# PhilippKath/concentus

Hardware: NVIDIA B200
Metric: CELT decode audio-sec per sec (x realtime), 48k stereo (higher is better)
Workload: dtype int32

## Files before the change

concentus_b200/csrc/celt_arith.cuh:

```cuda
#pragma once
#include "celt_simt.cuh"

namespace cb {

typedef int16_t s16_t;

CB_DEV int s16(int x) { return (int)(int16_t)x; }
CB_DEV int imin(int a, int b) { return a < b ? a : b; }
CB_DEV int imax(int a, int b) { return a > b ? a : b; }
CB_DEV int iabs(int a) { return a < 0 ? -a : a; }
CB_DEV int wadd(int a, int b) { return (int)((unsigned)a + (unsigned)b); }
CB_DEV int wsub(int a, int b) { return (int)((unsigned)a - (unsigned)b); }
CB_DEV int wmul(int a, int b) { return (int)((unsigned)a * (unsigned)b); }
CB_DEV int wneg(int a) { return (int)(0u - (unsigned)a); }

CB_DEV int ec_ilog(unsigned x) { return 32 - CB_CLZ(x); }

CB_DEV int shl32(int a, int s) { return (int)((unsigned)a << s); }
CB_DEV int shr32(int a, int s) { return a >> s; }
CB_DEV int pshr32(int a, int s) { return wadd(a, (1 << s) >> 1) >> s; }
CB_DEV int vshr32(int a, int s) { return s > 0 ? (a >> s) : shl32(a, -s); }
CB_DEV int shl16(int a, int s) { return s16((int)((unsigned)(uint16_t)a << s)); }
CB_DEV int round16(int a, int s) { return s16(pshr32(a, s)); }
CB_DEV int sat16(int x) { return x > 32767 ? 32767 : (x < -32768 ? -32768 : x); }

CB_DEV int mul16_16(int a, int b) { return s16(a) * s16(b); }
CB_DEV int mac16_16(int c, int a, int b) { return wadd(c, s16(a) * s16(b)); }
CB_DEV int mul16_16_q15(int a, int b) { return mul16_16(a, b) >> 15; }
CB_DEV int mul16_16_q14(int a, int b) { return mul16_16(a, b) >> 14; }
CB_DEV int mul16_16_q13(int a, int b) { return mul16_16(a, b) >> 13; }
CB_DEV int mul16_16_q11(int a, int b) { return mul16_16(a, b) >> 11; }
CB_DEV int mul16_16_p15(int a, int b) { return wadd(16384, mul16_16(a, b)) >> 15; }
CB_DEV int mul16_16_p14(int a, int b) { return wadd(8192, mul16_16(a, b)) >> 14; }
CB_DEV int mul16_16_p13(int a, int b) { return wadd(4096, mul16_16(a, b)) >> 13; }

CB_DEV int mul16_32_q15(int a, int b) { return (int)(((int64_t)s16(a) * (int64_t)b) >> 15); }
CB_DEV int mul16_32_q16(int a, int b) { return (int)(((int64_t)s16(a) * (int64_t)b) >> 16); }
CB_DEV int mul16_32_p16(int a, int b) { return (int)(((int64_t)s16(a) * (int64_t)b + 32768) >> 16); }
CB_DEV int mul32_32_q31(int a, int b) {
    int ah = a >> 16, bh = b >> 16;
    int al = a & 0xffff, bl = b & 0xffff;
    int t0 = shl32(s16(ah) * s16(bh), 1);
    int t1 = (s16(ah) * bl) >> 15;
    int t2 = (s16(bh) * al) >> 15;
    return wadd(wadd(t0, t1), t2);
}
CB_DEV int mac16_32_q15(int c, int a, int b) {
    return wadd(c, wadd(s16(a) * s16(b >> 15), (s16(a) * (b & 0x7fff)) >> 15));
}
CB_DEV int frac_mul16(int a, int b) { return (16384 + s16(a) * s16(b)) >> 15; }
CB_DEV int sig2word16(int x) { return sat16(pshr32(x, 12)); }

CB_DEV int celt_ilog2(int x) { return ec_ilog((unsigned)x) - 1; }
CB_DEV int celt_zlog2(int x) { return x <= 0 ? 0 : celt_ilog2(x); }

CB_MATH unsigned isqrt32(unsigned v) {
    unsigned g = 0;
    int bshift = (ec_ilog(v) - 1) >> 1;
    unsigned b = 1u << bshift;
    do {
        unsigned t = ((g << 1) + b) << bshift;
        if (t <= v) { g += b; v -= t; }
        b >>= 1;
        bshift--;
    } while (bshift >= 0);
    return g;
}

CB_MATH int celt_rcp(int x) {
    int i = celt_ilog2(x);
    int n = s16(vshr32(x, i - 15) - 32768);
    int r = s16(30840 + mul16_16_q15(-15420, n));
    r = s16(r - mul16_16_q15(r, s16(mul16_16_q15(r, n) + s16(r - 32768))));
    r = s16(r - s16(1 + mul16_16_q15(r, s16(mul16_16_q15(r, n) + s16(r - 32768)))));
    return vshr32(r, i - 16);
}
CB_DEV int celt_div(int a, int b) { return mul32_32_q31(a, celt_rcp(b)); }

CB_MATH int frac_div32(int a, int b) {
    int shift = celt_ilog2(b) - 29;
    a = vshr32(a, shift);
    b = vshr32(b, shift);
    int rcp = round16(celt_rcp(round16(b, 16)), 3);
    int result = mul16_32_q15(rcp, a);
    int rem = wsub(pshr32(a, 2), mul32_32_q31(result, b));
    result = wadd(result, shl32(mul16_32_q15(rcp, rem), 2));
    if (result >= 536870912) return 2147483647;
    if (result <= -536870912) return -2147483647;
    return shl32(result, 2);
}

CB_MATH int celt_rsqrt_norm(int x) {
    int n = s16(x - 32768);
    int r = s16(23557 + mul16_16_q15(n, s16(-13490 + mul16_16_q15(n, 6713))));
    int r2 = s16(mul16_16_q15(r, r));
    int y = shl16(s16(s16(mul16_16_q15(r2, n) + r2)) - 16384, 1);
    return s16(r + mul16_16_q15(r, s16(mul16_16_q15(y, s16(s16(mul16_16_q15(y, 12288)) - 16384)))));
}

CB_MATH int celt_sqrt(int x) {
    if (x == 0) return 0;
    if (x >= 1073741824) return 32767;
    int k = (celt_ilog2(x) >> 1) - 7;
    x = vshr32(x, 2 * k);
    int n = s16(x - 32768);
    int rt = s16(23175 + mul16_16_q15(n, s16(11561 + mul16_16_q15(n, s16(-3011 +
              mul16_16_q15(n, s16(1699 + mul16_16_q15(n, -664))))))));
    return vshr32(rt, 7 - k);
}

CB_MATH int celt_cos_pi_2(int x) {
    int x2 = s16(mul16_16_p15(x, x));
    int inner = wadd(-7651, mul16_16_p15(x2, wadd(8277, mul16_16_p15(-626, x2))));
    int v = wadd((32767 - x2), mul16_16_p15(x2, inner));
    return s16(1 + imin(32766, v));
}
CB_MATH int celt_cos_norm(int x) {
    x = x & 0x0001ffff;
    if (x > (1 << 16)) x = (1 << 17) - x;
    if (x & 0x00007fff) {
        if (x < (1 << 15)) return celt_cos_pi_2(s16(x));
        return s16(-celt_cos_pi_2(s16(65536 - x)));
    }
    if (x & 0x0000ffff) return 0;
    if (x & 0x0001ffff) return -32767;
    return 32767;
}

CB_MATH int celt_log2(int x) {
    if (x == 0) return -32767;
    int i = celt_ilog2(x);
    int n = s16(vshr32(x, i - 15) - 32768 - 16384);
    int frac = s16(-6793 + mul16_16_q15(n, s16(15746 + mul16_16_q15(n, s16(-5217 +
                mul16_16_q15(n, s16(2545 + mul16_16_q15(n, -1401))))))));
    return s16(shl16(i - 13, 10) + (frac >> 4));
}

CB_DEV int celt_exp2_frac(int x) {
    int frac = shl16(x, 4);
    return s16(16383 + mul16_16_q15(frac, s16(22804 + mul16_16_q15(frac, s16(14819 + mul16_16_q15(10204, frac))))));
}
CB_MATH int celt_exp2(int x) {
    int integer = s16(x) >> 10;
    if (integer > 14) return 0x7f000000;
    if (integer < -15) return 0;
    int frac = celt_exp2_frac(s16(s16(x) - shl16(integer, 10)));
    return vshr32(frac, -integer - 2);
}

CB_DEV int celt_atan01(int x) {
    return s16(mul16_16_p15(x, wadd(32767, mul16_16_p15(x, wadd(-21, mul16_16_p15(x, wadd(-11943, mul16_16_p15(4936, x))))))));
}
CB_MATH int celt_atan2p(int y, int x) {
    if (y < x) {
        int arg = celt_div(shl32(y, 15), x);
        if (arg >= 32767) arg = 32767;
        return celt_atan01(s16(arg)) >> 1;
    } else {
        int arg = celt_div(shl32(x, 15), y);
        if (arg >= 32767) arg = 32767;
        return 25736 - (celt_atan01(s16(arg)) >> 1);
    }
}

CB_MATH int bitexact_cos(int x) {
    x = s16(x);
    int tmp = (4096 + x * x) >> 13;
    int x2 = s16(tmp);
    x2 = s16((32767 - x2) + frac_mul16(x2, (-7651 + frac_mul16(x2, (8277 + frac_mul16(-626, x2))))));
    return s16(1 + x2);
}
CB_MATH int bitexact_log2tan(int isin, int icos) {
    int lc = ec_ilog((unsigned)icos);
    int ls = ec_ilog((unsigned)isin);
    icos <<= 15 - lc;
    isin <<= 15 - ls;
    return (ls - lc) * (1 << 11) + frac_mul16(isin, frac_mul16(isin, -2597) + 7932)
           - frac_mul16(icos, frac_mul16(icos, -2597) + 7932);
}

CB_DEV unsigned lcg_rand(unsigned seed) { return 1664525u * seed + 1013904223u; }
CB_TABLE uint32_t kLcgMul[23] = {1u, 1664525u, 389569705u, 2940799637u, 158984081u, 2862450781u, 3211393721u, 1851289957u, 3934847009u, 2184914861u, 246739401u, 1948736821u, 2941245873u, 4195587069u, 4088025561u, 980655621u, 2001863745u, 657792333u, 65284841u, 1282409429u, 3808694225u, 2968195997u, 2417331449u};
CB_TABLE uint32_t kLcgAdd[23] = {0u, 1013904223u, 1196435762u, 3519870697u, 2868466484u, 1649599747u, 2670642822u, 1476291629u, 2748932008u, 2180890343u, 2498801434u, 3421909937u, 3167820124u, 2636375307u, 3801544430u, 28987765u, 2210837584u, 3039689583u, 1338634754u, 1649346937u, 2768872580u, 2254235155u, 2326606934u};
CB_DEV unsigned lcg_jump(unsigned seed, int k) { return kLcgMul[k] * seed + kLcgAdd[k]; }

CB_DEV unsigned udiv(unsigned n, unsigned d) { return n / d; }
CB_DEV int sudiv(int n, int d) { return n / d; }

}
```

concentus_b200/csrc/celt_decoder.cuh:

```cuda
#pragma once
#include "celt_bands.cuh"
#include "celt_energy.cuh"
#include "celt_ir.h"
#include "celt_mdct.cuh"
#include "opus_state.h"


namespace cb {


struct ParseScratch {
    int16_t norm[2 * 8 * 78];
    alignas(16) int16_t tmp[176];
    alignas(16) int16_t xw[2 * 176];
    alignas(16) int16_t lbs[176];
};

CB_DEV void celt_parse_frame(const uint8_t *data, int len, int LM, int C, int end, unsigned *seed, CbFrameIR &ir, int16_t *X,
                             ParseScratch &ps, bool dry) {
    const int start = 0;
    const int M = 1 << LM;
    const int N = M * kShortMdct;
    int tf_res[kNbEBands], cap[kNbEBands], offsets[kNbEBands], fine_quant[kNbEBands], pulses[kNbEBands], fine_priority[kNbEBands];
    AllocScratch alloc;
    EcDec dec;
    dec.init(data, (unsigned)len);

    int total_bits = len * 8;
    int tell = dec.tell();
    int silence;
    if (tell >= total_bits) silence = 1;
    else if (tell == 1) silence = dec.bit_logp(15);
    else silence = 0;
    if (silence) {
        tell = len * 8;
        dec.nbits_total += tell - dec.tell();
    }
    int postfilter_gain = 0, postfilter_pitch = 0, postfilter_tapset = 0;
    if (start == 0 && tell + 16 <= total_bits) {
        if (dec.bit_logp(1)) {
            int octave = (int)dec.uint_(6);
            postfilter_pitch = (16 << octave) + (int)dec.bits(4 + octave) - 1;
            int qg = (int)dec.bits(3);
            if (dec.tell() + 2 <= total_bits) postfilter_tapset = dec.icdf(kTapsetIcdf, 2);
            postfilter_gain = 3072 * (qg + 1);
        }
        tell = dec.tell();
    }
    int isTransient = 0;
    if (LM > 0 && tell + 3 <= total_bits) {
        isTransient = dec.bit_logp(3);
        tell = dec.tell();
    }
    const int shortBlocks = isTransient ? M : 0;
    const int intra_ener = tell + 3 <= total_bits ? dec.bit_logp(3) : 0;
    CB_NOUNROLL for (int i = 0; i < 2 * kNbEBands; i++) { ir.qi[i] = 0; ir.eoff[i] = 0; }
    decode_coarse_symbols(start, end, intra_ener, dec, C, LM, ir.qi);
    tf_decode(start, end, isTransient, tf_res, LM, dec);
    tell = dec.tell();
    int spread_decision = kSpreadNormal;
    if (tell + 4 <= total_bits) spread_decision = dec.icdf(kSpreadIcdf, 5);
    init_caps(cap, LM, C);
    int dynalloc_logp = 6;
    total_bits <<= kBitRes;
    tell = (int)dec.tell_frac();
    CB_NOUNROLL for (int i = start; i < end; i++) {
        int width = C * band_width(i) << LM;
        int quanta = imin(width << kBitRes, imax(6 << kBitRes, width));
        int loop_logp = dynalloc_logp;
        int boost = 0;
        while (tell + (loop_logp << kBitRes) < total_bits && boost < cap[i]) {
            int flag = dec.bit_logp(loop_logp);
            tell = (int)dec.tell_frac();
            if (!flag) break;
            boost += quanta;
            total_bits -= quanta;
            loop_logp = 1;
        }
        offsets[i] = boost;
        if (boost > 0) dynalloc_logp = imax(2, dynalloc_logp - 1);
    }
    int alloc_trim = tell + (6 << kBitRes) <= total_bits ? dec.icdf(kTrimIcdf, 7) : 5;
    int bits = ((len * 8) << kBitRes) - (int)dec.tell_frac() - 1;
    int anti_collapse_rsv = isTransient && LM >= 2 && bits >= ((LM + 2) << kBitRes) ? (1 << kBitRes) : 0;
    bits -= anti_collapse_rsv;
    int intensity = 0, dual_stereo = 0, balance = 0;
    AllocDecIo io{dec};
    int codedBands = compute_allocation(io, alloc, start, end, offsets, cap, alloc_trim, &intensity, &dual_stereo, bits, &balance,
                                        pulses, fine_quant, fine_priority, C, LM);
    decode_fine_energy(start, end, fine_quant, dec, C, ir.eoff);

    unsigned sd = *seed;
    quant_all_bands_dec(start, end, X, C == 2 ? X + N : nullptr, ir.collapse, pulses, shortBlocks, spread_decision, dual_stereo,
                        intensity, tf_res, len * (8 << kBitRes) - anti_collapse_rsv, balance, dec, LM, codedBands, &sd, ps.norm,
                        ps.tmp, ps.xw, ps.lbs, dry);
    int anti_collapse_on = 0;
    if (anti_collapse_rsv > 0) anti_collapse_on = (int)dec.bits(1);
    decode_energy_finalise(start, end, fine_quant, fine_priority, len * 8 - dec.tell(), dec, C, ir.eoff);

    ir.rng_final = dec.rng;
    ir.seed_bands = sd;
    ir.len = (int16_t)len;
    ir.pf_pitch = (int16_t)postfilter_pitch;
    ir.pf_gain = (int16_t)postfilter_gain;
    ir.pf_tapset = (uint8_t)postfilter_tapset;
    ir.LM = (uint8_t)LM; ir.C = (uint8_t)C; ir.end = (uint8_t)end;
    ir.flags = (uint8_t)((silence ? CB_IR_SILENCE : 0) | (isTransient ? CB_IR_TRANSIENT : 0) | (intra_ener ? CB_IR_INTRA : 0) |
                         (anti_collapse_on ? CB_IR_ANTICOLLAPSE : 0) | (dec.error ? CB_IR_EC_ERROR : 0) |
                         (dec.tell() > 8 * len ? CB_IR_OVERRUN : 0));
    CB_NOUNROLL for (int i = 0; i < kNbEBands; i++) ir.pulses[i] = (int16_t)(i < end ? pulses[i] : 0);
    *seed = dec.rng;
}


struct SynthScratch {
    int fft[kMaxFrame];
    int16_t den_gain[2][kNbEBands];
    int8_t den_shift[2][kNbEBands];
};

template <class TM>
CB_DEV void comb_filter_inplace(TM tm, int *x, int T0, int T1, int N, int g0, int g1, int tapset0, int tapset1, int overlap) {
    if (g0 == 0 && g1 == 0) return;
    const int g00 = s16(mul16_16_p15(g0, kCombGains[tapset0][0]));
    const int g01 = s16(mul16_16_p15(g0, kCombGains[tapset0][1]));
    const int g02 = s16(mul16_16_p15(g0, kCombGains[tapset0][2]));
    const int g10 = s16(mul16_16_p15(g1, kCombGains[tapset1][0]));
    const int g11 = s16(mul16_16_p15(g1, kCombGains[tapset1][1]));
    const int g12 = s16(mul16_16_p15(g1, kCombGains[tapset1][2]));
    if (g0 == g1 && T0 == T1 && tapset0 == tapset1) overlap = 0;
    const int Tmin = imin(g0 != 0 ? T0 : kCombMaxPeriod, g1 != 0 ? T1 : kCombMaxPeriod);
    const int G = imin(TM::W, Tmin - 2);
    CB_NOUNROLL for (int base = 0; base < overlap; base += G) {
        int i = base + tm.lane();
        if (tm.lane() < G && i < overlap) {
            int f = s16(mul16_16_q15(kWindow120[i], kWindow120[i]));
            int nf = 32767 - f;
            int v = x[i];
            if (g0 != 0) {
                v = wadd(v, mul16_32_q15(mul16_16_q15(nf, g00), x[i - T0]));
                v = wadd(v, mul16_32_q15(mul16_16_q15(nf, g01), wadd(x[i - T0 + 1], x[i - T0 - 1])));
                v = wadd(v, mul16_32_q15(mul16_16_q15(nf, g02), wadd(x[i - T0 + 2], x[i - T0 - 2])));
            }
            if (g1 != 0) {
                v = wadd(v, mul16_32_q15(mul16_16_q15(f, g10), x[i - T1]));
                v = wadd(v, mul16_32_q15(mul16_16_q15(f, g11), wadd(x[i - T1 + 1], x[i - T1 - 1])));
                v = wadd(v, mul16_32_q15(mul16_16_q15(f, g12), wadd(x[i - T1 + 2], x[i - T1 - 2])));
            }
            x[i] = v;
        }
        tm.sync();
    }
    if (g1 == 0) return;
    CB_NOUNROLL for (int base = overlap; base < N; base += G) {
        int i = base + tm.lane();
        if (tm.lane() < G && i < N) {
            int v = x[i];
            v = wadd(v, mul16_32_q15(g10, x[i - T1]));
            v = wadd(v, mul16_32_q15(g11, wadd(x[i - T1 + 1], x[i - T1 - 1])));
            v = wadd(v, mul16_32_q15(g12, wadd(x[i - T1 + 2], x[i - T1 - 2])));
            x[i] = v;
        }
        tm.sync();
    }
}

CB_DEV int deemphasis_channel(const int *x, int n, int16_t *y, int CC, int downsample, int m, int gain) {
    if (downsample > 1) {
        int k = 0, next = 0;
        CB_NOUNROLL for (int j = 0; j < n; j++) {
            int t = wadd(x[j], m);
            m = mul16_32_q15(kPreemphCoef0, t);
            if (j == next) {
                int v = sig2word16(t);
                if (gain >= 0) { int g = mul16_32_p16(v, gain); v = g > 32767 ? 32767 : (g < -32767 ? -32767 : g); }
                y[k * CC] = (int16_t)v;
                k++;
                next += downsample;
            }
        }
    } else {
        int j = 0;
        if ((((uintptr_t)x) & 15) == 0) {
            CB_NOUNROLL for (; j + 8 <= n; j += 8) {
                int xs[8];
                const int4 a = *reinterpret_cast<const int4 *>(x + j);
                const int4 b = *reinterpret_cast<const int4 *>(x + j + 4);
                xs[0] = a.x; xs[1] = a.y; xs[2] = a.z; xs[3] = a.w; xs[4] = b.x; xs[5] = b.y; xs[6] = b.z; xs[7] = b.w;
#pragma unroll
                CB_NOUNROLL for (int u = 0; u < 8; u++) {
                    int t = wadd(xs[u], m);
                    m = mul16_32_q15(kPreemphCoef0, t);
                    int v = sig2word16(t);
                    if (gain >= 0) { int g = mul16_32_p16(v, gain); v = g > 32767 ? 32767 : (g < -32767 ? -32767 : g); }
                    y[(j + u) * CC] = (int16_t)v;
                }
            }
        }
        CB_NOUNROLL for (; j < n; j++) {
            int t = wadd(x[j], m);
            m = mul16_32_q15(kPreemphCoef0, t);
            int v = sig2word16(t);
            if (gain >= 0) { int g = mul16_32_p16(v, gain); v = g > 32767 ? 32767 : (g < -32767 ? -32767 : g); }
            y[j * CC] = (int16_t)v;
        }
    }
    return m;
}

template <class TM>
CB_DEV void history_shift(TM tm, int *mem, int N, int count = -1) {
    if (count < 0) count = kDecBuf - N + kOverlap / 2;
    if (((count | N) & 3) == 0) {
        int4 *m4 = reinterpret_cast<int4 *>(mem);
        const int nv = count >> 2, sh = N >> 2;
        CB_NOUNROLL for (int base = 0; base < nv; base += 2 * TM::W) {
            const int i0 = base + tm.lane(), i1 = i0 + TM::W;
            int4 a = {0, 0, 0, 0}, b = {0, 0, 0, 0};
            if (i0 < nv) a = m4[i0 + sh];
            if (i1 < nv) b = m4[i1 + sh];
            tm.sync();
            if (i0 < nv) m4[i0] = a;
            if (i1 < nv) m4[i1] = b;
        }
        tm.sync();
        return;
    }
    CB_NOUNROLL for (int base = 0; base < count; base += TM::W) {
        int i = base + tm.lane();
        int v = 0;
        if (i < count) v = mem[i + N];
        tm.sync();
        if (i < count) mem[i] = v;
    }
    tm.sync();
}

template <class TM>
CB_DEV void celt_synthesis_team(TM tm, SynthScratch &S, const int16_t *X, int *const *out_syn, const int16_t *oldBandE, int start, int effEnd,
                                int C, int CC, int isTransient, int LM, int downsample, int silence) {
    const int M = 1 << LM;
    const int N = M * kShortMdct;
    {
        int bstart = start, bend = effEnd;
        int bound = M * kEBands[bend];
        if (downsample != 1) bound = imin(bound, N / downsample);
        if (silence) { bound = 0; bstart = bend = 0; }
        const int lo = M * kEBands[bstart];
        CB_TEAM_FOR(w, C * kNbEBands, tm) {
            int c = w / kNbEBands, i = w - c * kNbEBands;
            int lg = s16(oldBandE[c * kNbEBands + i] + shl16(kEMeans[i], 6));
            int shift = 16 - (lg >> 10);
            int g;
            if (shift > 31) { shift = 0; g = 0; }
            else g = celt_exp2_frac(lg & 1023);
            if (shift < -2) { g = 32767; shift = -2; }
            S.den_gain[c][i] = (int16_t)g;
            S.den_shift[c][i] = (int8_t)shift;
        }
        tm.sync();
        const int B = isTransient ? M : 1;
        const int shift = isTransient ? kMaxLM : kMaxLM - LM;
        const int hi = imin(bound, M * kEBands[bend]);
        auto freq = [&](int mode, int j) -> int {
            if (j < lo || j >= hi) return 0;
            const int b = kBinToBand[j >> LM];
            int v0 = 0, v1 = 0;
            if (mode != 1) {
                int v = mul16_16(X[j], S.den_gain[0][b]);
                int sh = S.den_shift[0][b];
                v0 = sh < 0 ? shl32(v, -sh) : (v >> sh);
            }
            if (mode != 0) {
                int v = mul16_16(X[N + j], S.den_gain[1][b]);
                int sh = S.den_shift[1][b];
                v1 = sh < 0 ? shl32(v, -sh) : (v >> sh);
            }
            return mode == 0 ? v0 : mode == 1 ? v1 : (wadd(v0, v1) >> 1);
        };
        const int npass = (CC == 2 && C == 2) ? 2 : 1;
        CB_NOUNROLL for (int p = 0; p < npass; p++) {
            const int mode = (CC == 1 && C == 2) ? 2 : p;
            imdct_compute(tm, [&](int j) { return freq(mode, j); }, B, shift, S.fft);
            imdct_assemble(tm, out_syn[p], B, shift, S.fft);
            if (CC == 2 && C == 1) imdct_assemble(tm, out_syn[1], B, shift, S.fft);
        }
    }
}

template <class TM>
CB_DEV int celt_synth_frame(TM tm, CbDecState *st, SynthScratch &S, const CbFrameIR &ir, int16_t *X, int *const *sig) {
    const int CC = st->channels;
    const int LM = ir.LM, C = ir.C, end = ir.end, start = 0;
    const int M = 1 << LM;
    const int N = M * kShortMdct;
    const int silence = ir.flags & CB_IR_SILENCE, isTransient = (ir.flags & CB_IR_TRANSIENT) != 0;
    int *decode_mem[2], *out_syn[2];
    CB_NOUNROLL for (int c = 0; c < CC; c++) {
        decode_mem[c] = st->decode_mem + c * CB_DEC_MEM;
        out_syn[c] = decode_mem[c] + kDecBuf - N;
    }
    const int effEnd = imin(end, kNbEBands);
    int16_t *oldBandE = st->oldEBands, *oldLogE = st->oldLogE, *oldLogE2 = st->oldLogE2, *backgroundLogE = st->backgroundLogE;

    if (tm.lane() == 0) {
        if (C == 1)
            CB_NOUNROLL for (int i = 0; i < kNbEBands; i++) oldBandE[i] = (int16_t)imax(oldBandE[i], oldBandE[kNbEBands + i]);
        apply_coarse_energy(start, end, oldBandE, ir.qi, (ir.flags & CB_IR_INTRA) != 0, C, LM);
        CB_NOUNROLL for (int c = 0; c < C; c++)
            CB_NOUNROLL for (int i = start; i < end; i++)
                oldBandE[c * kNbEBands + i] = (int16_t)(oldBandE[c * kNbEBands + i] + ir.eoff[c * kNbEBands + i]);
    }
    tm.sync();
    CB_NOUNROLL for (int c = 0; c < CC; c++) history_shift(tm, decode_mem[c], N);
    if (ir.flags & CB_IR_ANTICOLLAPSE)
        anti_collapse(tm, X, ir.collapse, LM, C, N, start, end, oldBandE, oldLogE, oldLogE2, ir.pulses, ir.seed_bands);
    if (silence) {
        CB_TEAM_FOR(i, C * kNbEBands, tm) oldBandE[i] = -28672;
        tm.sync();
    }

    celt_synthesis_team(tm, S, X, out_syn, oldBandE, start, effEnd, C, CC, isTransient, LM, st->downsample, silence);

    const int pf_period = imax(st->postfilter_period, kCombMinPeriod);
    const int pf_period_old = imax(st->postfilter_period_old, kCombMinPeriod);
    const int postfilter_pitch = ir.pf_pitch, postfilter_gain = ir.pf_gain, postfilter_tapset = ir.pf_tapset;
    CB_NOUNROLL for (int c = 0; c < CC; c++) {
        comb_filter_inplace(tm, out_syn[c], pf_period_old, pf_period, kShortMdct, st->postfilter_gain_old, st->postfilter_gain,
                            st->postfilter_tapset_old, st->postfilter_tapset, kOverlap);
        if (LM != 0)
            comb_filter_inplace(tm, out_syn[c] + kShortMdct, pf_period, postfilter_pitch, N - kShortMdct, st->postfilter_gain,
                                postfilter_gain, st->postfilter_tapset, postfilter_tapset, kOverlap);
    }
    tm.sync();
    if (tm.lane() == 0) {
        st->postfilter_period_old = pf_period;
        st->postfilter_gain_old = st->postfilter_gain;
        st->postfilter_tapset_old = st->postfilter_tapset;
        st->postfilter_period = postfilter_pitch;
        st->postfilter_gain = postfilter_gain;
        st->postfilter_tapset = postfilter_tapset;
        if (LM != 0) {
            st->postfilter_period_old = st->postfilter_period;
            st->postfilter_gain_old = st->postfilter_gain;
            st->postfilter_tapset_old = st->postfilter_tapset;
        }
        if (C == 1)
            CB_NOUNROLL for (int i = 0; i < kNbEBands; i++) oldBandE[kNbEBands + i] = oldBandE[i];
        if (!isTransient) {
            const int max_inc = st->loss_count < 10 ? M : 1024;
            CB_NOUNROLL for (int i = 0; i < 2 * kNbEBands; i++) {
                oldLogE2[i] = oldLogE[i];
                oldLogE[i] = oldBandE[i];
                backgroundLogE[i] = (int16_t)imin(backgroundLogE[i] + max_inc, (int)oldBandE[i]);
            }
        } else {
            CB_NOUNROLL for (int i = 0; i < 2 * kNbEBands; i++) oldLogE[i] = (int16_t)imin(oldLogE[i], oldBandE[i]);
        }
        CB_NOUNROLL for (int c = 0; c < 2; c++) {
            CB_NOUNROLL for (int i = 0; i < start; i++) {
                oldBandE[c * kNbEBands + i] = 0;
                oldLogE[c * kNbEBands + i] = oldLogE2[c * kNbEBands + i] = -28672;
            }
            CB_NOUNROLL for (int i = end; i < kNbEBands; i++) {
                oldBandE[c * kNbEBands + i] = 0;
                oldLogE[c * kNbEBands + i] = oldLogE2[c * kNbEBands + i] = -28672;
            }
        }
        st->rng = ir.rng_final;
        st->loss_count = 0;
        if (ir.flags & CB_IR_EC_ERROR) st->error = 1;
    }
    tm.sync();
    CB_NOUNROLL for (int c = 0; c < CC; c++) {
        const int *src = out_syn[c];
        int *dst = sig[c];
        CB_TEAM_FOR(j, N, tm) dst[j] = src[j];
    }
    tm.sync();
    if (ir.flags & CB_IR_OVERRUN) return OPUS_INTERNAL_ERROR_;
    return N / st->downsample;
}

}
```

concentus_b200/csrc/celt_mdct.cuh:

```cuda
#pragma once
#include "celt_arith.cuh"
#include "celt_tables.cuh"

namespace cb {

struct Cpx { int r, i; };

CB_DEV int smul(int x, int tw) { return mul16_32_q15(tw, x); }
CB_DEV Cpx cmul(Cpx a, int twr, int twi) {
    Cpx m;
    m.r = wsub(smul(a.r, twr), smul(a.i, twi));
    m.i = wadd(smul(a.r, twi), smul(a.i, twr));
    return m;
}
CB_DEV Cpx cadd(Cpx a, Cpx b) { Cpx c; c.r = wadd(a.r, b.r); c.i = wadd(a.i, b.i); return c; }
CB_DEV Cpx csub(Cpx a, Cpx b) { Cpx c; c.r = wsub(a.r, b.r); c.i = wsub(a.i, b.i); return c; }
CB_DEV void tw_load(int idx, int &r, int &i) {
    unsigned w = kFftTwiddles[idx];
    r = (int)(int16_t)(w & 0xffff);
    i = (int)(int16_t)(w >> 16);
}

template <class TM>
CB_DEV void fft_inplace(TM tm, Cpx *buf, int s, int nblocks) {
    const FftPlan &pl = kFftPlan[s];
    const int nfft = pl.nfft;
    CB_NOUNROLL for (int st = 0; st < pl.nstages; st++) {
        const int p = pl.radix[st];
        const int m = pl.m[st];
        const int mm = p * m;
        const int ngroups = nfft / mm;
        const int fs = ngroups << pl.tw_shift;
        if (p == 2) {
            const int items = nblocks * ngroups * 4;
            CB_TEAM_FOR(w, items, tm) {
                int q = w & 3, g = w >> 2;
                int blk = g / ngroups, grp = g - blk * ngroups;
                Cpx *F = buf + blk * nfft + grp * 8 + q;
                Cpx a = F[0], b = F[4], t;
                if (q == 0) t = b;
                else if (q == 1) { t.r = smul(wadd(b.r, b.i), 23170); t.i = smul(wsub(b.i, b.r), 23170); }
                else if (q == 2) { t.r = b.i; t.i = wneg(b.r); }
                else { t.r = smul(wsub(b.i, b.r), 23170); t.i = smul(wsub(wneg(b.i), b.r), 23170); }
                F[4] = csub(a, t);
                F[0] = cadd(a, t);
            }
        } else if (p == 4 && m == 1) {
            const int items = nblocks * ngroups;
            CB_TEAM_FOR(w, items, tm) {
                int blk = w / ngroups, grp = w - blk * ngroups;
                Cpx *F = buf + blk * nfft + grp * 4;
                Cpx f0 = F[0], f1 = F[1], f2 = F[2], f3 = F[3];
                Cpx s0 = csub(f0, f2);
                f0 = cadd(f0, f2);
                Cpx s1 = cadd(f1, f3);
                f2 = csub(f0, s1);
                f0 = cadd(f0, s1);
                s1 = csub(f1, f3);
                F[0] = f0;
                F[2] = f2;
                Cpx o1, o3;
                o1.r = wadd(s0.r, s1.i); o1.i = wsub(s0.i, s1.r);
                o3.r = wsub(s0.r, s1.i); o3.i = wadd(s0.i, s1.r);
                F[1] = o1;
                F[3] = o3;
            }
        } else if (p == 4) {
            const int items = nblocks * ngroups * m;
            CB_TEAM_FOR(w, items, tm) {
                int j = w % m, g = w / m;
                int blk = g / ngroups, grp = g - blk * ngroups;
                Cpx *F = buf + blk * nfft + grp * mm + j;
                int r1, i1, r2, i2, r3, i3;
                tw_load(j * fs, r1, i1);
                tw_load(2 * j * fs, r2, i2);
                tw_load(3 * j * fs, r3, i3);
                Cpx f0 = F[0];
                Cpx c0 = cmul(F[m], r1, i1);
                Cpx c1 = cmul(F[2 * m], r2, i2);
                Cpx c2 = cmul(F[3 * m], r3, i3);
                Cpx c5 = csub(f0, c1);
                f0 = cadd(f0, c1);
                Cpx c3 = cadd(c0, c2);
                Cpx c4 = csub(c0, c2);
                F[2 * m] = csub(f0, c3);
                F[0] = cadd(f0, c3);
                Cpx o1, o3;
                o1.r = wadd(c5.r, c4.i); o1.i = wsub(c5.i, c4.r);
                o3.r = wsub(c5.r, c4.i); o3.i = wadd(c5.i, c4.r);
                F[m] = o1;
                F[3 * m] = o3;
            }
        } else if (p == 3) {
            const int items = nblocks * ngroups * m;
            CB_TEAM_FOR(w, items, tm) {
                int j = w % m, g = w / m;
                int blk = g / ngroups, grp = g - blk * ngroups;
                Cpx *F = buf + blk * nfft + grp * mm + j;
                int r1, i1, r2, i2;
                tw_load(j * fs, r1, i1);
                tw_load(2 * j * fs, r2, i2);
                Cpx f0 = F[0];
                Cpx c1 = cmul(F[m], r1, i1);
                Cpx c2 = cmul(F[2 * m], r2, i2);
                Cpx c3 = cadd(c1, c2);
                Cpx c0 = csub(c1, c2);
                Cpx fm;
                fm.r = wsub(f0.r, c3.r >> 1);
                fm.i = wsub(f0.i, c3.i >> 1);
                c0.r = smul(c0.r, -28378);
                c0.i = smul(c0.i, -28378);
                F[0] = cadd(f0, c3);
                Cpx o2, o1;
                o2.r = wadd(fm.r, c0.i); o2.i = wsub(fm.i, c0.r);
                o1.r = wsub(fm.r, c0.i); o1.i = wadd(fm.i, c0.r);
                F[2 * m] = o2;
                F[m] = o1;
            }
        } else {
            const int items = nblocks * ngroups * m;
            CB_TEAM_FOR(w, items, tm) {
                int u = w % m, g = w / m;
                int blk = g / ngroups, grp = g - blk * ngroups;
                Cpx *F = buf + blk * nfft + grp * mm + u;
                int r1, i1, r2, i2, r3, i3, r4, i4;
                tw_load(u * fs, r1, i1);
                tw_load(2 * u * fs, r2, i2);
                tw_load(3 * u * fs, r3, i3);
                tw_load(4 * u * fs, r4, i4);
                Cpx s0 = F[0];
                Cpx s1 = cmul(F[m], r1, i1);
                Cpx s2 = cmul(F[2 * m], r2, i2);
                Cpx s3 = cmul(F[3 * m], r3, i3);
                Cpx s4 = cmul(F[4 * m], r4, i4);
                Cpx s7 = cadd(s1, s4), s10 = csub(s1, s4);
                Cpx s8 = cadd(s2, s3), s9 = csub(s2, s3);
                Cpx o0;
                o0.r = wadd(s0.r, wadd(s7.r, s8.r));
                o0.i = wadd(s0.i, wadd(s7.i, s8.i));
                F[0] = o0;
                Cpx s5, s6, s11, s12;
                s5.r = wadd(wadd(s0.r, smul(s7.r, 10126)), smul(s8.r, -26510));
                s5.i = wadd(wadd(s0.i, smul(s7.i, 10126)), smul(s8.i, -26510));
                s6.r = wadd(smul(s10.i, -31164), smul(s9.i, -19261));
                s6.i = wsub(wneg(smul(s10.r, -31164)), smul(s9.r, -19261));
                F[m] = csub(s5, s6);
                F[4 * m] = cadd(s5, s6);
                s11.r = wadd(wadd(s0.r, smul(s7.r, -26510)), smul(s8.r, 10126));
                s11.i = wadd(wadd(s0.i, smul(s7.i, -26510)), smul(s8.i, 10126));
                s12.r = wadd(wneg(smul(s10.i, -19261)), smul(s9.i, -31164));
                s12.i = wsub(smul(s10.r, -19261), smul(s9.r, -31164));
                F[2 * m] = cadd(s11, s12);
                F[3 * m] = csub(s11, s12);
            }
        }
        tm.sync();
    }
}

template <class TM, class FreqFn>
CB_DEV void imdct_compute(TM tm, FreqFn freq, int B, int shift, int *fftbuf) {
    const int N2 = (kMaxFrame * 2 >> shift) >> 1;
    const int N4 = N2 >> 1;
    int trig_off = 0;
    CB_NOUNROLL for (int i = 0, n = kMaxFrame * 2; i < shift; i++) { n >>= 1; trig_off += n; }
    const int16_t *t = kMdctTwiddles + trig_off;
    const int16_t *bitrev = fft_bitrev(shift);
    CB_TEAM_FOR(w, B * N4, tm) {
        int b = w / N4, i = w - b * N4;
        int x1 = freq(b + (2 * i) * B);
        int x2 = freq(b + (N2 - 1 - 2 * i) * B);
        int t0 = t[i], t1 = t[N4 + i];
        int yr = wadd(smul(x2, t0), smul(x1, t1));
        int yi = wsub(smul(x1, t0), smul(x2, t1));
        int rev = bitrev[i];
        fftbuf[b * N2 + 2 * rev + 1] = yr;
        fftbuf[b * N2 + 2 * rev] = yi;
    }
    tm.sync();
    fft_inplace(tm, (Cpx *)fftbuf, shift, B);
    CB_TEAM_FOR(w, B * ((N4 + 1) >> 1), tm) {
        int half = (N4 + 1) >> 1;
        int b = w / half, i = w - b * half;
        int *yp0 = fftbuf + b * N2 + 2 * i;
        int *yp1 = fftbuf + b * N2 + N2 - 2 - 2 * i;
        int re = yp0[1], im = yp0[0];
        int t0 = t[i], t1 = t[N4 + i];
        int yr = wadd(smul(re, t0), smul(im, t1));
        int yi = wsub(smul(re, t1), smul(im, t0));
        re = yp1[1];
        im = yp1[0];
        yp0[0] = yr;
        yp1[1] = yi;
        t0 = t[N4 - i - 1];
        t1 = t[N2 - i - 1];
        yr = wadd(smul(re, t0), smul(im, t1));
        yi = wsub(smul(re, t1), smul(im, t0));
        yp1[0] = yr;
        yp0[1] = yi;
    }
    tm.sync();
}

template <class TM>
CB_DEV void imdct_assemble(TM tm, int *out, int B, int shift, const int *fftbuf) {
    const int N2 = (kMaxFrame * 2 >> shift) >> 1;
    const int N = B * N2;
    const int half = kOverlap >> 1;
    CB_TEAM_FOR(j, N + half, tm) {
        int b = j / N2;
        int r = j - b * N2;
        if (b < B && r < kOverlap) {
            if (r < half) {
                int i = r;
                int x2 = b == 0 ? out[i] : fftbuf[(b - 1) * N2 + (N2 - half) + i];
                int x1 = fftbuf[b * N2 + (half - 1 - i)];
                int lo = wsub(smul(x2, kWindow120[kOverlap - 1 - i]), smul(x1, kWindow120[i]));
                int hi = wadd(smul(x2, kWindow120[i]), smul(x1, kWindow120[kOverlap - 1 - i]));
                out[b * N2 + i] = lo;
                out[b * N2 + kOverlap - 1 - i] = hi;
            }
        } else {
            int bb = b < B ? b : B - 1;
            int k = j - bb * N2 - half;
            out[j] = fftbuf[bb * N2 + k];
        }
    }
    tm.sync();
}

template <class TM>
CB_DEV void mdct_forward(TM tm, const int *in, int *out, int shift, int stride, int *f, int *f2) {
    const int N2 = (kMaxFrame * 2 >> shift) >> 1;
    const int N4 = N2 >> 1;
    int trig_off = 0;
    CB_NOUNROLL for (int i = 0, n = kMaxFrame * 2; i < shift; i++) { n >>= 1; trig_off += n; }
    const int16_t *t = kMdctTwiddles + trig_off;
    const int16_t *bitrev = fft_bitrev(shift);
    const FftPlan &pl = kFftPlan[shift];
    const int scale_shift = pl.scale_shift - 1;
    const int ov = kOverlap, q = (ov + 3) >> 2;
    CB_TEAM_FOR(i, N4, tm) {
        const int *xp1 = in + (ov >> 1) + 2 * i;
        const int *xp2 = in + N2 - 1 + (ov >> 1) - 2 * i;
        int re, im;
        if (i < q) {
            const int w1 = kWindow120[(ov >> 1) + 2 * i], w2 = kWindow120[(ov >> 1) - 1 - 2 * i];
            re = wadd(smul(xp1[N2], w2), smul(*xp2, w1));
            im = wsub(smul(*xp1, w1), smul(xp2[-N2], w2));
        } else if (i < N4 - q) {
            re = *xp2;
            im = *xp1;
        } else {
            const int k = i - (N4 - q);
            const int w1 = kWindow120[2 * k], w2 = kWindow120[ov - 1 - 2 * k];
            re = wadd(wneg(smul(xp1[-N2], w1)), smul(*xp2, w2));
            im = wadd(smul(*xp1, w2), smul(xp2[N2], w1));
        }
        f[2 * i] = re;
        f[2 * i + 1] = im;
    }
    tm.sync();
    CB_TEAM_FOR(i, N4, tm) {
        const int t0 = t[i], t1 = t[N4 + i];
        const int re = f[2 * i], im = f[2 * i + 1];
        int yr = wsub(smul(re, t0), smul(im, t1));
        int yi = wadd(smul(im, t0), smul(re, t1));
        yr = pshr32(mul16_32_q16(kFftScale, yr), scale_shift);
        yi = pshr32(mul16_32_q16(kFftScale, yi), scale_shift);
        const int rev = bitrev[i];
        f2[2 * rev] = yr;
        f2[2 * rev + 1] = yi;
    }
    tm.sync();
    fft_inplace(tm, (Cpx *)f2, shift, 1);
    CB_TEAM_FOR(i, N4, tm) {
        const int fr = f2[2 * i], fi = f2[2 * i + 1];
        const int yr = wsub(smul(fi, t[N4 + i]), smul(fr, t[i]));
        const int yi = wadd(smul(fr, t[N4 + i]), smul(fi, t[i]));
        out[stride * (2 * i)] = yr;
        out[stride * (N2 - 1 - 2 * i)] = yi;
    }
    tm.sync();
}

}
```

Measured before the change: 159,700.

## Fuse output copy into IMDCT/comb filter, precompute denorm table, use fast division

Writes the synthesized samples straight to the output signal during IMDCT assembly and comb filtering, which removes the separate copy pass at the end. Band denormalization is folded into a per-bin gain/shift table so each frequency lookup avoids the band-index lookup and branches. Integer divisions in the FFT and IMDCT index math are replaced by multiply-high magic-number division, and the serial lane-0 energy bookkeeping loops are spread across the team. The cost is extra stores and scratch space, and the magic-number division is only exact for small index ranges.

Measured after the change: 176,200 (median of 6 runs). 1.1x the previous value.

```diff
diff --git a/concentus_b200/csrc/celt_arith.cuh b/concentus_b200/csrc/celt_arith.cuh
--- a/concentus_b200/csrc/celt_arith.cuh
+++ b/concentus_b200/csrc/celt_arith.cuh
@@ -187,4 +187,11 @@
 CB_DEV unsigned udiv(unsigned n, unsigned d) { return n / d; }
 CB_DEV int sudiv(int n, int d) { return n / d; }
 
+CB_DEV unsigned fastdiv_magic(unsigned d) { return 0xffffffffu / d + 1u; }
+#if defined(__CUDACC__)
+CB_DEV int fastdiv(int n, unsigned magic) { return (int)__umulhi((unsigned)n, magic); }
+#else
+CB_DEV int fastdiv(int n, unsigned magic) { return (int)(((uint64_t)(unsigned)n * magic) >> 32); }
+#endif
+
 }
diff --git a/concentus_b200/csrc/celt_decoder.cuh b/concentus_b200/csrc/celt_decoder.cuh
--- a/concentus_b200/csrc/celt_decoder.cuh
+++ b/concentus_b200/csrc/celt_decoder.cuh
@@ -113,14 +113,18 @@
 }
 
 
+enum { kDenBins = 100 };
+
 struct SynthScratch {
     int fft[kMaxFrame];
     int16_t den_gain[2][kNbEBands];
     int8_t den_shift[2][kNbEBands];
+    int den[2][kDenBins];
 };
 
 template <class TM>
-CB_DEV void comb_filter_inplace(TM tm, int *x, int T0, int T1, int N, int g0, int g1, int tapset0, int tapset1, int overlap) {
+CB_DEV void comb_filter_inplace(TM tm, int *x, int T0, int T1, int N, int g0, int g1, int tapset0, int tapset1, int overlap,
+                                int *y = nullptr) {
     if (g0 == 0 && g1 == 0) return;
     const int g00 = s16(mul16_16_p15(g0, kCombGains[tapset0][0]));
     const int g01 = s16(mul16_16_p15(g0, kCombGains[tapset0][1]));
@@ -148,6 +152,7 @@
                 v = wadd(v, mul16_32_q15(mul16_16_q15(f, g12), wadd(x[i - T1 + 2], x[i - T1 - 2])));
             }
             x[i] = v;
+            if (y) y[i] = v;
         }
         tm.sync();
     }
@@ -160,6 +165,7 @@
             v = wadd(v, mul16_32_q15(g11, wadd(x[i - T1 + 1], x[i - T1 - 1])));
             v = wadd(v, mul16_32_q15(g12, wadd(x[i - T1 + 2], x[i - T1 - 2])));
             x[i] = v;
+            if (y) y[i] = v;
         }
         tm.sync();
     }
@@ -238,53 +244,53 @@
 
 template <class TM>
 CB_DEV void celt_synthesis_team(TM tm, SynthScratch &S, const int16_t *X, int *const *out_syn, const int16_t *oldBandE, int start, int effEnd,
-                                int C, int CC, int isTransient, int LM, int downsample, int silence) {
+                                int C, int CC, int isTransient, int LM, int downsample, int silence, int *const *sig = nullptr) {
     const int M = 1 << LM;
     const int N = M * kShortMdct;
-    {
-        int bstart = start, bend = effEnd;
-        int bound = M * kEBands[bend];
-        if (downsample != 1) bound = imin(bound, N / downsample);
-        if (silence) { bound = 0; bstart = bend = 0; }
-        const int lo = M * kEBands[bstart];
-        CB_TEAM_FOR(w, C * kNbEBands, tm) {
-            int c = w / kNbEBands, i = w - c * kNbEBands;
-            int lg = s16(oldBandE[c * kNbEBands + i] + shl16(kEMeans[i], 6));
-            int shift = 16 - (lg >> 10);
-            int g;
-            if (shift > 31) { shift = 0; g = 0; }
-            else g = celt_exp2_frac(lg & 1023);
-            if (shift < -2) { g = 32767; shift = -2; }
-            S.den_gain[c][i] = (int16_t)g;
-            S.den_shift[c][i] = (int8_t)shift;
-        }
-        tm.sync();
-        const int B = isTransient ? M : 1;
-        const int shift = isTransient ? kMaxLM : kMaxLM - LM;
-        const int hi = imin(bound, M * kEBands[bend]);
-        auto freq = [&](int mode, int j) -> int {
-            if (j < lo || j >= hi) return 0;
-            const int b = kBinToBand[j >> LM];
-            int v0 = 0, v1 = 0;
-            if (mode != 1) {
-                int v = mul16_16(X[j], S.den_gain[0][b]);
-                int sh = S.den_shift[0][b];
-                v0 = sh < 0 ? shl32(v, -sh) : (v >> sh);
-            }
-            if (mode != 0) {
-                int v = mul16_16(X[N + j], S.den_gain[1][b]);
-                int sh = S.den_shift[1][b];
-                v1 = sh < 0 ? shl32(v, -sh) : (v >> sh);
-            }
-            return mode == 0 ? v0 : mode == 1 ? v1 : (wadd(v0, v1) >> 1);
-        };
-        const int npass = (CC == 2 && C == 2) ? 2 : 1;
-        CB_NOUNROLL for (int p = 0; p < npass; p++) {
-            const int mode = (CC == 1 && C == 2) ? 2 : p;
-            imdct_compute(tm, [&](int j) { return freq(mode, j); }, B, shift, S.fft);
-            imdct_assemble(tm, out_syn[p], B, shift, S.fft);
-            if (CC == 2 && C == 1) imdct_assemble(tm, out_syn[1], B, shift, S.fft);
-        }
+    int bstart = start, bend = effEnd;
+    int bound = M * kEBands[bend];
+    if (downsample != 1) bound = imin(bound, N / downsample);
+    if (silence) { bound = 0; bstart = bend = 0; }
+    CB_TEAM_FOR(w, C * kNbEBands, tm) {
+        int c = w / kNbEBands, i = w - c * kNbEBands;
+        int lg = s16(oldBandE[c * kNbEBands + i] + shl16(kEMeans[i], 6));
+        int shift = 16 - (lg >> 10);
+        int g;
+        if (shift > 31) { shift = 0; g = 0; }
+        else g = celt_exp2_frac(lg & 1023);
+        if (shift < -2) { g = 32767; shift = -2; }
+        S.den_gain[c][i] = (int16_t)g;
+        S.den_shift[c][i] = (int8_t)shift;
+    }
+    tm.sync();
+    CB_TEAM_FOR(w, C * kDenBins, tm) {
+        const int c = w >= kDenBins, k = w - c * kDenBins;
+        const int b = kBinToBand[k];
+        int e = 0;
+        if (b >= bstart && b < bend) {
+            const int sh = S.den_shift[c][b];
+            e = ((int)S.den_gain[c][b] << (imax(-sh, 0) + 5)) | imax(sh, 0);
+        }
+        S.den[c][k] = e;
+    }
+    tm.sync();
+    const int B = isTransient ? M : 1;
+    const int shift = isTransient ? kMaxLM : kMaxLM - LM;
+    const int hi = imin(bound, M * kEBands[bend]);
+    auto den = [&](int c, int j) -> int {
+        const int e = S.den[c][j >> LM];
+        return wmul(X[c * N + j], e >> 5) >> (e & 31);
+    };
+    auto freq = [&](int mode, int j) -> int {
+        if (j >= hi) return 0;
+        return mode != 2 ? den(mode, j) : (wadd(den(0, j), den(1, j)) >> 1);
+    };
+    const int npass = (CC == 2 && C == 2) ? 2 : 1;
+    CB_NOUNROLL for (int p = 0; p < npass; p++) {
+        const int mode = (CC == 1 && C == 2) ? 2 : p;
+        imdct_compute(tm, [&](int j) { return freq(mode, j); }, B, shift, S.fft);
+        imdct_assemble(tm, out_syn[p], B, shift, S.fft, sig ? sig[p] : nullptr);
+        if (CC == 2 && C == 1) imdct_assemble(tm, out_syn[1], B, shift, S.fft, sig ? sig[1] : nullptr);
     }
 }
 
@@ -307,9 +313,11 @@
         if (C == 1)
             CB_NOUNROLL for (int i = 0; i < kNbEBands; i++) oldBandE[i] = (int16_t)imax(oldBandE[i], oldBandE[kNbEBands + i]);
         apply_coarse_energy(start, end, oldBandE, ir.qi, (ir.flags & CB_IR_INTRA) != 0, C, LM);
-        CB_NOUNROLL for (int c = 0; c < C; c++)
-            CB_NOUNROLL for (int i = start; i < end; i++)
-                oldBandE[c * kNbEBands + i] = (int16_t)(oldBandE[c * kNbEBands + i] + ir.eoff[c * kNbEBands + i]);
+    }
+    tm.sync();
+    CB_TEAM_FOR(w, C * kNbEBands, tm) {
+        const int i = w >= kNbEBands ? w - kNbEBands : w;
+        if (i >= start && i < end) oldBandE[w] = (int16_t)(oldBandE[w] + ir.eoff[w]);
     }
     tm.sync();
     CB_NOUNROLL for (int c = 0; c < CC; c++) history_shift(tm, decode_mem[c], N);
@@ -320,17 +328,18 @@
         tm.sync();
     }
 
-    celt_synthesis_team(tm, S, X, out_syn, oldBandE, start, effEnd, C, CC, isTransient, LM, st->downsample, silence);
+    celt_synthesis_team(tm, S, X, out_syn, oldBandE, start, effEnd, C, CC, isTransient, LM, st->downsample, silence, sig);
 
     const int pf_period = imax(st->postfilter_period, kCombMinPeriod);
     const int pf_period_old = imax(st->postfilter_period_old, kCombMinPeriod);
     const int postfilter_pitch = ir.pf_pitch, postfilter_gain = ir.pf_gain, postfilter_tapset = ir.pf_tapset;
+    const int max_inc = st->loss_count < 10 ? M : 1024;
     CB_NOUNROLL for (int c = 0; c < CC; c++) {
         comb_filter_inplace(tm, out_syn[c], pf_period_old, pf_period, kShortMdct, st->postfilter_gain_old, st->postfilter_gain,
-                            st->postfilter_tapset_old, st->postfilter_tapset, kOverlap);
+                            st->postfilter_tapset_old, st->postfilter_tapset, kOverlap, sig[c]);
         if (LM != 0)
             comb_filter_inplace(tm, out_syn[c] + kShortMdct, pf_period, postfilter_pitch, N - kShortMdct, st->postfilter_gain,
-                                postfilter_gain, st->postfilter_tapset, postfilter_tapset, kOverlap);
+                                postfilter_gain, st->postfilter_tapset, postfilter_tapset, kOverlap, sig[c] + kShortMdct);
     }
     tm.sync();
     if (tm.lane() == 0) {
@@ -345,37 +354,28 @@
             st->postfilter_gain_old = st->postfilter_gain;
             st->postfilter_tapset_old = st->postfilter_tapset;
         }
-        if (C == 1)
-            CB_NOUNROLL for (int i = 0; i < kNbEBands; i++) oldBandE[kNbEBands + i] = oldBandE[i];
-        if (!isTransient) {
-            const int max_inc = st->loss_count < 10 ? M : 1024;
-            CB_NOUNROLL for (int i = 0; i < 2 * kNbEBands; i++) {
-                oldLogE2[i] = oldLogE[i];
-                oldLogE[i] = oldBandE[i];
-                backgroundLogE[i] = (int16_t)imin(backgroundLogE[i] + max_inc, (int)oldBandE[i]);
-            }
-        } else {
-            CB_NOUNROLL for (int i = 0; i < 2 * kNbEBands; i++) oldLogE[i] = (int16_t)imin(oldLogE[i], oldBandE[i]);
-        }
-        CB_NOUNROLL for (int c = 0; c < 2; c++) {
-            CB_NOUNROLL for (int i = 0; i < start; i++) {
-                oldBandE[c * kNbEBands + i] = 0;
-                oldLogE[c * kNbEBands + i] = oldLogE2[c * kNbEBands + i] = -28672;
-            }
-            CB_NOUNROLL for (int i = end; i < kNbEBands; i++) {
-                oldBandE[c * kNbEBands + i] = 0;
-                oldLogE[c * kNbEBands + i] = oldLogE2[c * kNbEBands + i] = -28672;
-            }
-        }
         st->rng = ir.rng_final;
         st->loss_count = 0;
         if (ir.flags & CB_IR_EC_ERROR) st->error = 1;
     }
-    tm.sync();
-    CB_NOUNROLL for (int c = 0; c < CC; c++) {
-        const int *src = out_syn[c];
-        int *dst = sig[c];
-        CB_TEAM_FOR(j, N, tm) dst[j] = src[j];
+    if (C == 1) {
+        CB_TEAM_FOR(i, kNbEBands, tm) oldBandE[kNbEBands + i] = oldBandE[i];
+        tm.sync();
+    }
+    CB_TEAM_FOR(w, 2 * kNbEBands, tm) {
+        const int i = w >= kNbEBands ? w - kNbEBands : w;
+        const int e = oldBandE[w];
+        if (!isTransient) {
+            oldLogE2[w] = oldLogE[w];
+            oldLogE[w] = (int16_t)e;
+            backgroundLogE[w] = (int16_t)imin(backgroundLogE[w] + max_inc, e);
+        } else {
+            oldLogE[w] = (int16_t)imin(oldLogE[w], e);
+        }
+        if (i < start || i >= end) {
+            oldBandE[w] = 0;
+            oldLogE[w] = oldLogE2[w] = -28672;
+        }
     }
     tm.sync();
     if (ir.flags & CB_IR_OVERRUN) return OPUS_INTERNAL_ERROR_;
diff --git a/concentus_b200/csrc/celt_mdct.cuh b/concentus_b200/csrc/celt_mdct.cuh
--- a/concentus_b200/csrc/celt_mdct.cuh
+++ b/concentus_b200/csrc/celt_mdct.cuh
@@ -35,8 +35,7 @@
             const int items = nblocks * ngroups * 4;
             CB_TEAM_FOR(w, items, tm) {
                 int q = w & 3, g = w >> 2;
-                int blk = g / ngroups, grp = g - blk * ngroups;
-                Cpx *F = buf + blk * nfft + grp * 8 + q;
+                Cpx *F = buf + g * 8 + q;
                 Cpx a = F[0], b = F[4], t;
                 if (q == 0) t = b;
                 else if (q == 1) { t.r = smul(wadd(b.r, b.i), 23170); t.i = smul(wsub(b.i, b.r), 23170); }
@@ -48,8 +47,7 @@
         } else if (p == 4 && m == 1) {
             const int items = nblocks * ngroups;
             CB_TEAM_FOR(w, items, tm) {
-                int blk = w / ngroups, grp = w - blk * ngroups;
-                Cpx *F = buf + blk * nfft + grp * 4;
+                Cpx *F = buf + w * 4;
                 Cpx f0 = F[0], f1 = F[1], f2 = F[2], f3 = F[3];
                 Cpx s0 = csub(f0, f2);
                 f0 = cadd(f0, f2);
@@ -67,10 +65,10 @@
             }
         } else if (p == 4) {
             const int items = nblocks * ngroups * m;
-            CB_TEAM_FOR(w, items, tm) {
-                int j = w % m, g = w / m;
-                int blk = g / ngroups, grp = g - blk * ngroups;
-                Cpx *F = buf + blk * nfft + grp * mm + j;
+            const unsigned mmag = fastdiv_magic(m);
+            CB_TEAM_FOR(w, items, tm) {
+                int g = fastdiv(w, mmag), j = w - g * m;
+                Cpx *F = buf + w + g * (mm - m);
                 int r1, i1, r2, i2, r3, i3;
                 tw_load(j * fs, r1, i1);
                 tw_load(2 * j * fs, r2, i2);
@@ -93,10 +91,10 @@
             }
         } else if (p == 3) {
             const int items = nblocks * ngroups * m;
-            CB_TEAM_FOR(w, items, tm) {
-                int j = w % m, g = w / m;
-                int blk = g / ngroups, grp = g - blk * ngroups;
-                Cpx *F = buf + blk * nfft + grp * mm + j;
+            const unsigned mmag = fastdiv_magic(m);
+            CB_TEAM_FOR(w, items, tm) {
+                int g = fastdiv(w, mmag), j = w - g * m;
+                Cpx *F = buf + w + g * (mm - m);
                 int r1, i1, r2, i2;
                 tw_load(j * fs, r1, i1);
                 tw_load(2 * j * fs, r2, i2);
@@ -119,10 +117,10 @@
             }
         } else {
             const int items = nblocks * ngroups * m;
-            CB_TEAM_FOR(w, items, tm) {
-                int u = w % m, g = w / m;
-                int blk = g / ngroups, grp = g - blk * ngroups;
-                Cpx *F = buf + blk * nfft + grp * mm + u;
+            const unsigned mmag = fastdiv_magic(m);
+            CB_TEAM_FOR(w, items, tm) {
+                int g = fastdiv(w, mmag), u = w - g * m;
+                Cpx *F = buf + w + g * (mm - m);
                 int r1, i1, r2, i2, r3, i3, r4, i4;
                 tw_load(u * fs, r1, i1);
                 tw_load(2 * u * fs, r2, i2);
@@ -166,8 +164,9 @@
     CB_NOUNROLL for (int i = 0, n = kMaxFrame * 2; i < shift; i++) { n >>= 1; trig_off += n; }
     const int16_t *t = kMdctTwiddles + trig_off;
     const int16_t *bitrev = fft_bitrev(shift);
+    const unsigned n4mag = fastdiv_magic(N4), halfmag = fastdiv_magic(N4 >> 1);
     CB_TEAM_FOR(w, B * N4, tm) {
-        int b = w / N4, i = w - b * N4;
+        int b = fastdiv(w, n4mag), i = w - b * N4;
         int x1 = freq(b + (2 * i) * B);
         int x2 = freq(b + (N2 - 1 - 2 * i) * B);
         int t0 = t[i], t1 = t[N4 + i];
@@ -179,9 +178,8 @@
     }
     tm.sync();
     fft_inplace(tm, (Cpx *)fftbuf, shift, B);
-    CB_TEAM_FOR(w, B * ((N4 + 1) >> 1), tm) {
-        int half = (N4 + 1) >> 1;
-        int b = w / half, i = w - b * half;
+    CB_TEAM_FOR(w, B * (N4 >> 1), tm) {
+        int b = fastdiv(w, halfmag), i = w - b * (N4 >> 1);
         int *yp0 = fftbuf + b * N2 + 2 * i;
         int *yp1 = fftbuf + b * N2 + N2 - 2 - 2 * i;
         int re = yp0[1], im = yp0[0];
@@ -203,12 +201,13 @@
 }
 
 template <class TM>
-CB_DEV void imdct_assemble(TM tm, int *out, int B, int shift, const int *fftbuf) {
+CB_DEV void imdct_assemble(TM tm, int *out, int B, int shift, const int *fftbuf, int *sig = nullptr) {
     const int N2 = (kMaxFrame * 2 >> shift) >> 1;
     const int N = B * N2;
     const int half = kOverlap >> 1;
+    const unsigned n2mag = fastdiv_magic(N2);
     CB_TEAM_FOR(j, N + half, tm) {
-        int b = j / N2;
+        int b = fastdiv(j, n2mag);
         int r = j - b * N2;
         if (b < B && r < kOverlap) {
             if (r < half) {
@@ -219,11 +218,17 @@
                 int hi = wadd(smul(x2, kWindow120[i]), smul(x1, kWindow120[kOverlap - 1 - i]));
                 out[b * N2 + i] = lo;
                 out[b * N2 + kOverlap - 1 - i] = hi;
+                if (sig) {
+                    sig[b * N2 + i] = lo;
+                    sig[b * N2 + kOverlap - 1 - i] = hi;
+                }
             }
         } else {
             int bb = b < B ? b : B - 1;
             int k = j - bb * N2 - half;
-            out[j] = fftbuf[bb * N2 + k];
+            const int v = fftbuf[bb * N2 + k];
+            out[j] = v;
+            if (sig && j < N) sig[j] = v;
         }
     }
     tm.sync();
```
